# RainbowXXX/3DReconstruction

Hardware: AMD Instinct MI355X
Metric: BA LM-iters/sec + obs/sec, 1k cams/500k pts/5M obs; SIFT match pairs/sec (higher is better)
Workload: dtype f64; 1 GPU; C4 BA 1000 cams / 500000 pts / 5000000 obs, banded orbit visibility k=10, HuberLoss(4), gauge image 1, Ceres-default LM to termination per step; parallelism=landmark-sharded x1, all-reduce of the RCS, transport=none

## Files before the change

3dreconstruction_amd/_abi.py:

```python
import ctypes as C
import os

_HERE = os.path.dirname(os.path.abspath(__file__))
LIB_PATH = os.path.join(_HERE, "lib", "libsfmcore.so")

SFM_OK = 0
SFM_ERR_INVALID_ARG = -1
SFM_ERR_DEVICE = -2
SFM_ERR_NOT_FINITE = -3
SFM_ERR_UNSUPPORTED = -4
SFM_ERR_COMM = -5
SFM_ERR_OOM = -6
SFM_ERR_SOLVER = -7

SFM_TERM_CONVERGENCE = 0
SFM_TERM_NO_CONVERGENCE = 1
SFM_TERM_FAILURE = 2

SFM_CAM_PINHOLE = 0
SFM_CAM_SNAVELY = 1
SFM_CAM_RADIAL3 = 2

SFM_CTX_TUNE_HOST_MALLOC = 1
SFM_CTX_DIAG_NO_EXCHANGE = 2
SFM_CTX_DIAG_FAIL_SOLVE_WAIT = 4
SFM_CTX_TIME_KERNELS = 8
SFM_CTX_BA_DENSE_RCS = 1 << 4
SFM_CTX_BA_SEQ_BAND = 1 << 5
SFM_CTX_BA_TILE80 = 1 << 6
SFM_CTX_BA_SPLIT_REDUCE = 1 << 7
SFM_CTX_BA_SPLIT_BCR = 1 << 8
SFM_CTX_BA_NO_SPEC_GRAM = 1 << 10
SFM_CTX_DIAG_SPEC_ALWAYS = 1 << 11
SFM_CTX_BA_DENSE_CHAIN = 1 << 9


def SFM_CTX_BA_STEP_LANES(n):
    return {1: 1, 2: 2, 4: 3, 8: 4}[n] << 12


def SFM_CTX_BA_REDUCE_WAVES(n):
    return {1: 1, 2: 2, 4: 3}[n] << 15


SFM_RCS_BCR, SFM_RCS_DENSE, SFM_RCS_SEQ_BAND = 0, 1, 2

SFM_TRI_LINEAR, SFM_TRI_ROBUST = 0, 1
SFM_TRI_OK, SFM_TRI_SHORT, SFM_TRI_ANGLE, SFM_TRI_INFINITE = 0, 1, 2, 3

# ... 336 lines not shown
```

3dreconstruction_amd/csrc/ba_bcr.h:

```cpp
#pragma once
#include <hip/hip_runtime.h>

#include <vector>

#include "ba_kernels.h"

namespace sfm {

constexpr int kBcrM = 64;
constexpr int kBcrK = 10;

struct BcrArgs {
    int N = 0;
    int K = 0;
    int nrhs = 0;
    double *A = nullptr, *C = nullptr, *L = nullptr, *Wl = nullptr, *Wr = nullptr;
    double *R = nullptr, *Z = nullptr, *Y = nullptr, *part = nullptr, *fail = nullptr;
    unsigned* yflag = nullptr;
    unsigned long long* stamps = nullptr;
    bool split = false;
};

struct DenseArgs {
    int nt = 0;
    int64_t np = 0;
    double *A = nullptr, *X = nullptr, *b = nullptr, *y = nullptr, *x = nullptr, *fail = nullptr;
    unsigned* xflag = nullptr;
    unsigned* fflag = nullptr;
    unsigned long long* xg = nullptr;
    unsigned long long* stamps = nullptr;
    const int32_t* meta = nullptr;
    int nch = 0, ntask = 0;
    int64_t meta_words = 0;
    bool flow = false;
    bool chain = false;
};
size_t dense_flag_words(const DenseArgs& d);
void dense_setup(DenseArgs& d, const DevProblem& P);
std::vector<int32_t> dense_flow_plan(DenseArgs& d, const DevProblem& P, const std::vector<char>* exact = nullptr);
std::vector<char> dense_tile_pattern(const std::vector<ReduceTarget>& targets, int64_t nF, int nt);
size_t dense_doubles(const DenseArgs& d);
void dense_bind(DenseArgs& d, double* base);
void dense_solve(const DenseArgs& d, const DevProblem& P, double radius, hipStream_t s, unsigned epoch);

bool bcr_supported(const DevProblem& P);
void bcr_setup(BcrArgs& b, const DevProblem& P);
size_t bcr_doubles(const BcrArgs& b);
inline size_t bcr_y_granules(const BcrArgs& b) { return (size_t)b.N * 128; }
void bcr_bind(BcrArgs& b, double* base);
struct BcrCand {
    const double* extr;
    const double* intr;
    double* cand_extr;
    double* cand_intr;
    CamPre* cand_cp;
};
void bcr_solve(const BcrArgs& b, const DevProblem& P, double radius, hipStream_t s, unsigned epoch,
               const BcrCand& cand);

}
```

3dreconstruction_amd/csrc/ba_bcr.hip:

```cpp
#include <hip/hip_runtime.h>

#include <algorithm>
#include <cfloat>
#include <cmath>
#include <cstdlib>
#include <cstring>
#include <functional>
#include <type_traits>
#include <utility>

#include "ba_bcr.h"
#include "ba_cand.h"
#include "common.h"

#if defined(__HIP_DEVICE_COMPILE__) && !defined(__gfx950__)
#error "counter-form hand-offs (sc1 payloads + vmcnt drain + relaxed ticket) are written for gfx950 only"
#endif

namespace sfm {
namespace {

constexpr int M = kBcrM;
constexpr int LD = M + 1;
constexpr int NT = 256;
// ... 10 lines not shown

__device__ __forceinline__ int bcr_kM(const BcrArgs& b) { return b.K <= 9 ? 56 : b.K == 10 ? 60 : 64; }

__device__ __forceinline__ double clampd(double v, double lo, double hi) { return fmin(fmax(v, lo), hi); }

typedef __attribute__((address_space(1))) unsigned long long gu64;
typedef __attribute__((address_space(1))) unsigned gu32;
typedef __attribute__((address_space(1))) double gf64;
__device__ __forceinline__ void st_sc1(double* p, double v) {
    __hip_atomic_store((gf64*)p, v, __ATOMIC_RELAXED, __HIP_MEMORY_SCOPE_AGENT);
}
__device__ __forceinline__ double ld_sc1(const double* p) {
    return __hip_atomic_load((gf64*)p, __ATOMIC_RELAXED, __HIP_MEMORY_SCOPE_AGENT);
}

typedef double v4d __attribute__((ext_vector_type(4)));

__device__ __forceinline__ unsigned long long stamp() {
    unsigned long long t;
    asm volatile("s_memtime %0\n\ts_waitcnt lgkmcnt(0)" : "=s"(t)::"memory");
    return t;
}

__device__ __forceinline__ void wave_sync() {
    __builtin_amdgcn_fence(__ATOMIC_RELEASE, "wavefront");
    __builtin_amdgcn_wave_barrier();
    __builtin_amdgcn_fence(__ATOMIC_ACQUIRE, "wavefront");
}

__device__ __forceinline__ double rsqrt_nr(double d) {
    const double y = __builtin_amdgcn_rsq(d);
// ... 67 lines not shown
    __builtin_amdgcn_sched_barrier(0);
#pragma unroll
    for (int q = 0; q < 16; ++q)
        if (q < 14 || 4 * q < kM) acc = __builtin_amdgcn_mfma_f64_16x16x4f64(NEG ? -a[q] : a[q], b[q], acc, 0, 0, 0);
    return acc;
}
struct GTile {
    double v[16];
    __device__ __forceinline__ void fetch(const double* p, int ld) {
        const int lane = threadIdx.x & 63, i = lane & 15, kk = lane >> 4;
#pragma unroll
        for (int c = 0; c < 4; ++c)
#pragma unroll
            for (int j = 0; j < 4; ++j) v[4 * c + j] = p[(16 * c + 4 * j + kk) * ld + i];
    }
};
template <bool NEG, class PA>
__device__ __forceinline__ v4d mm_tr(v4d acc, PA A, int lda, int ar, const GTile& g, int kM) {
    const int lane = threadIdx.x & 63, i = lane & 15, kk = lane >> 4;
    double a[16];
#pragma unroll
    for (int q = 0; q < 16; ++q) a[q] = A[(4 * q + kk) * lda + ar + i];
    __builtin_amdgcn_sched_barrier(0);
#pragma unroll
    for (int q = 0; q < 16; ++q)
        if (q < 14 || 4 * q < kM)
            acc = __builtin_amdgcn_mfma_f64_16x16x4f64(NEG ? -a[q] : a[q], g.v[q], acc, 0, 0, 0);
    return acc;
}
template <bool NEG, class PB>
// ... 10 lines not shown
    return acc;
}
__device__ __forceinline__ lds_cd* L3(const double* p) { return (lds_cd*)p; }

__device__ __forceinline__ v4d tile_ld(const double* C, int ldc, int r0, int c0) {
    const int lane = threadIdx.x & 63, i = lane & 15, kk = lane >> 4;
    v4d v;
#pragma unroll
    for (int r = 0; r < 4; ++r) v[r] = C[(r0 + kk + 4 * r) * ldc + c0 + i];
    return v;
}
__device__ __forceinline__ void tile_st(double* C, int ldc, int r0, int c0, v4d v) {
    const int lane = threadIdx.x & 63, i = lane & 15, kk = lane >> 4;
#pragma unroll
    for (int r = 0; r < 4; ++r) C[(r0 + kk + 4 * r) * ldc + c0 + i] = v[r];
}
__device__ __forceinline__ v4d zero4() { return v4d{0.0, 0.0, 0.0, 0.0}; }

template <int NC, int R = M, int TH = NT>
__device__ __forceinline__ void load_tile(double* dst, int ld_dst, const double* __restrict__ src, int ld_src) {
    constexpr int n2 = R * NC / 2, per = (n2 + TH - 1) / TH;
    double2 v[per];
#pragma unroll
    for (int q = 0; q < per; ++q) {
        const int e = threadIdx.x + q * TH;
        if (e < n2) v[q] = *reinterpret_cast<const double2*>(src + (e / (NC / 2)) * ld_src + 2 * (e % (NC / 2)));
    }
#pragma unroll
    for (int q = 0; q < per; ++q) {
        const int e = threadIdx.x + q * TH;
// ... 1 lines not shown
            double* d = dst + (e / (NC / 2)) * ld_dst + 2 * (e % (NC / 2));
            d[0] = v[q].x;
            d[1] = v[q].y;
        }
    }
}
template <int NC, int R = M, int TH = NT>
struct TileFetch {
    static constexpr int n2 = R * NC / 2, per = (n2 + TH - 1) / TH;
    double2 v[per];
    __device__ __forceinline__ void fetch(const double* __restrict__ src, int ld_src) {
#pragma unroll
        for (int q = 0; q < per; ++q) {
            const int e = threadIdx.x + q * TH;
            if (e < n2) v[q] = *reinterpret_cast<const double2*>(src + (e / (NC / 2)) * ld_src + 2 * (e % (NC / 2)));
        }
    }
    __device__ __forceinline__ void put(double* dst, int ld_dst) const {
#pragma unroll
        for (int q = 0; q < per; ++q) {
            const int e = threadIdx.x + q * TH;
            if (e < n2) {
                double* d = dst + (e / (NC / 2)) * ld_dst + 2 * (e % (NC / 2));
                d[0] = v[q].x;
                d[1] = v[q].y;
            }
        }
    }
};
__device__ __forceinline__ void load_tiles2(double* d1, const double* __restrict__ s1, double* d2,
// ... 297 lines not shown
        const double lm = sqrt(clampd(cn, P.min_diag, P.max_diag) / radius);
        dmp = creal ? lm * lm : 0.0;
    }
    __device__ __forceinline__ double a(const DevProblem& P, int r, int c) const {
        const int ci = c0 + r / 6, rm = r % 6;
        const bool real = r < nreal && creal;
        const int d = ci >= cj ? ci - cj : cj - ci;
        const bool inband = real && d <= P.D;
        const int idx = ci >= cj ? ((ci * Dp + d) * 36 + rm * 6 + cm) : ((cj * Dp + d) * 36 + cm * 6 + rm);
        const double v = P.Sband[inband ? idx : 0];
        double x = inband ? v : 0.0;
        x = (real && r == c) ? x + dmp : x;
        return r >= nreal && r == c ? 1.0 : x;
    }
};
template <int TH>
__device__ __forceinline__ void pack_rows(const BcrArgs& b, const DevProblem& P, double radius, int I, int r0, int t) {
    double* A = b.A + (size_t)I * M * M + (size_t)r0 * M;
    double* R = b.R + (size_t)I * M * b.nrhs + (size_t)r0 * b.nrhs;
    static_assert(TH % M == 0, "a thread's column is fixed");
    constexpr int NA = 16 * M / TH;
    const BandCol col(b, P, radius, I, t % M);
    double va[NA];
#pragma unroll
    for (int q = 0; q < NA; ++q) {
        const int e = t + q * TH;
        va[q] = col.a(P, r0 + e / M, e % M);
    }
    static_assert(16 * 32 <= TH, "one R element per thread at most (nrhs <= 32)");
    const bool hasr = t < 16 * b.nrhs;
    const double vr = pack_r(b, P, I, r0 + t / b.nrhs, t % b.nrhs, hasr);
#pragma unroll
    for (int q = 0; q < NA; ++q) A[t + q * TH] = va[q];
    if (hasr) R[t] = vr;
}

__global__ void bcr_pack_kernel(BcrArgs b, DevProblem P, double radius) {
    const int I = blockIdx.x >> 4, rg = blockIdx.x & 15;
    double* A = b.A + (size_t)I * M * M;
    double* Cm = b.C + (size_t)I * M * M;
    double* R = b.R + (size_t)I * M * b.nrhs;
    {
        const int e = 4 * rg * M + threadIdx.x;
        const int r = e / M, c = e % M;
        A[e] = pack_a(b, P, radius, I, r, c);
        Cm[e] = pack_c(b, P, I, r, c);
    }
    for (int e = 4 * rg * b.nrhs + threadIdx.x; e < 4 * (rg + 1) * b.nrhs; e += NT)
        R[e] = pack_r(b, P, I, e / b.nrhs, e % b.nrhs);
// ... 37 lines not shown
    if (wv < 4) {
        v4d acc = tile_ld(Aj, M, 16 * w, 16 * v);
        if (hl) acc = mm_ll_rows<true, false, true>(acc, L3(Wa), LD, 16 * w, L3(Wa), LD, 16 * v, kM);
        if (hr) acc = mm_ll_rows<true, false, true>(acc, L3(Wb), LD, 16 * w, L3(Wb), LD, 16 * v, kM);
        tile_st(Aj, M, 16 * w, 16 * v, acc);
        return;
    }
    if (16 * v < b.nrhs) {
        double* Rj = b.R + (size_t)j * M * b.nrhs;
        v4d acc = tile_ld(Rj, b.nrhs, 16 * w, 16 * v);
        if (hl) acc = mm_ll_rows<true, false, true>(acc, L3(Wa), LD, 16 * w, L3(Za), ldr, 16 * v, kM);
        if (hr) acc = mm_ll_rows<true, false, true>(acc, L3(Wb), LD, 16 * w, L3(Zb), ldr, 16 * v, kM);
        tile_st(Rj, b.nrhs, 16 * w, 16 * v, acc);
    }
}

constexpr int NTL = 512, NWL = NTL / 64;

__device__ __forceinline__ void bcr_corner_body(const BcrArgs& b, const DevProblem& P, double radius, int I,
                                                bool z_fresh, bool part_done = false, unsigned tag = 0,
                                                const double* own = nullptr);
__device__ __forceinline__ void put_y(unsigned long long* g, int row, double v, unsigned epoch);
__device__ __forceinline__ void corner_put_lds(const DevProblem& P, const v4d& q00, double* dst) {
    constexpr int kQ = 17;
    const int lane = threadIdx.x & 63, i = lane & 15, kk = lane >> 4, na = P.iw * P.nintr;
#pragma unroll
    for (int r = 0; r < 4; ++r) {
        const int ga = kk + 4 * r, gc = i;
        if (ga >= 1 && ga <= na && gc <= na) dst[(ga - 1) * kQ + gc] = q00[r];
    }
// ... 5 lines not shown
    double* out = b.part + (size_t)I * 512;
    auto put = [&](const v4d& q, int r0, int c0) {
#pragma unroll
        for (int r = 0; r < 4; ++r) {
            const int ga = r0 + kk + 4 * r, gc = c0 + i;
            if (ga >= 1 && ga <= na && gc <= na) st_sc1(out + (ga - 1) * kQ + gc, q[r]);
        }
    };
    put(q00, 0, 0);
    if (ntc > 1) {
        put(q10, 16, 0);
        put(q11, 16, 16);
    }
}

template <bool TOP>
__global__ __launch_bounds__(NTL) void bcr_level_kernel(BcrArgs b, DevProblem P, double radius, int s, int n_odd,
                                                        unsigned epoch) {
    extern __shared__ __attribute__((aligned(16))) double sm[];
    int item, w;
    if constexpr (TOP) {
        if ((int)blockIdx.x >= 4) {
            bcr_corner_body(b, P, radius, (int)blockIdx.x - 3, false, false, epoch);
            return;
        }
        item = 0;
        w = blockIdx.x;
    } else {
        const int xcd = blockIdx.x & 7, q = blockIdx.x >> 3;
        item = xcd + 8 * (q >> 2);
        w = q & 3;
    }
    const int sp = s >> 1;
    if (!TOP && item >= n_odd) {
        const int j = 2 * s * (item - n_odd);
        if (sp > 0 && j < b.N) update_tile_rows<NTL>(b, sp, j, w, sm);
        return;
    }
    const int i = TOP ? 0 : s + 2 * s * item;
    if (i >= b.N) return;
    const int r = i + s, wave = threadIdx.x >> 6;
    const bool hr = !TOP && r < b.N, hz = 16 * w < b.nrhs;
    const int np3 = 6 * b.K - 48;
    const int kM = bcr_kM(b);
    constexpr int L16 = 17;
    double* A = sm;
    double* X = A + M * LD;
    double* Wa_l = X + M * LD;
    double* Wb_l = Wa_l + M * M;
    double* Cc = Wb_l + M * M;
    double* Cr = Cc + M * L16;
    double* Rc = Cr + 16 * LD;
    double* bad = Rc + M * L16;
    double* col = bad + 2;
    unsigned* pdone = reinterpret_cast<unsigned*>(col + 16);
    unsigned long long* st = (b.stamps && w == 0 && !TOP) ? b.stamps : nullptr;
    unsigned long long t0 = 0, t1 = 0;
    if (st) t0 = stamp();
    if (threadIdx.x == 0) bad[0] = 0.0;
    if (threadIdx.x < 4) pdone[threadIdx.x] = 0u;
    TileFetch<64, M, NTL> fa;
    TileFetch<16, M, NTL> frc;
    if (!TOP && sp == 0) {
        constexpr int QA = M * M / NTL, QC = M * 16 / NTL;
        double va[QA], vc[QC], vr[QC], vz[QC];
        const BandCol col(b, P, radius, i, threadIdx.x % M);
#pragma unroll
        for (int q = 0; q < QA; ++q) {
            const int e = threadIdx.x + q * NTL;
            va[q] = col.a(P, e / M, e % M);
        }
// ... 4 lines not shown
            vr[q] = pack_c(b, P, r, 16 * w + e / M, e % M, hr);
            vz[q] = pack_r(b, P, i, e / 16, 16 * w + e % 16, hz);
        }
#pragma unroll
        for (int q = 0; q < QA; ++q) {
            const int e = threadIdx.x + q * NTL;
            A[(e / M) * LD + e % M] = va[q];
        }
#pragma unroll
        for (int q = 0; q < QC; ++q) {
            const int e = threadIdx.x + q * NTL;
            Cc[(e / 16) * L16 + e % 16] = vc[q];
            Cr[(e / M) * LD + e % M] = vr[q];
            Rc[(e / 16) * L16 + e % 16] = vz[q];
        }
        pack_rows<NTL>(b, P, radius, i - 1, 16 * w, threadIdx.x);
        if (i + 1 == b.N - 1) pack_rows<NTL>(b, P, radius, i + 1, 16 * w, threadIdx.x);
    } else {
        TileFetch<64, M, NTL> fwa, fwb;
        const bool hwb = i + sp < b.N;
        if (!TOP) fwa.fetch(b.Wr + (size_t)(i - sp) * M * M, M);
        if (hwb) fwb.fetch(b.Wl + (size_t)(i + sp) * M * M, M);
        fa.fetch(b.A + (size_t)i * M * M, M);
        if (hz) frc.fetch(b.R + (size_t)i * M * b.nrhs + 16 * w, b.nrhs);
        if (!TOP) fwa.put(Wa_l, M);
        if (hwb) fwb.put(Wb_l, M);
        fa.put(A, LD);
        if (hz) frc.put(Rc, L16);
    }
    __syncthreads();
    if (st) {
        t1 = stamp();
        if (threadIdx.x == 0) atomicAdd(st + 5, t1 - t0);
    }
    {
    const bool upd = sp > 0;
    const int il = TOP ? i : i - sp, ir = i + sp;
    const bool hir = upd && ir < b.N;
    const double* Z1 = b.Z + (size_t)il * M * b.nrhs + 16 * w;
// ... 37 lines not shown
    auto bgR = [&](int v, const GTile& g1, const GTile& g2) {
        if (!hzu) return;
        v4d acc = tile_ld(Rc, L16, 16 * v, 0);
        if (!TOP) acc = mm_tr<true>(acc, L3(Wal), M, 16 * v, g1, kM);
        if (hir) acc = mm_tr<true>(acc, L3(Wbl), M, 16 * v, g2, kM);
        tile_st(Rc, L16, 16 * v, 0, acc);
    };
    auto bgC = [&](int v, const GTile& gl) {
        if (upd && !TOP) tile_st(Cc, L16, 16 * v, 0, mm_tr<true>(zero4(), L3(Wal), M, 16 * v, gl, kM));
    };
    auto bgCr = [&](int v, const GTile& gr) {
        if (hr && hir) tile_st(Cr, LD, 0, 16 * v, mm_rt<true>(zero4(), gr, L3(Wbl), M, 16 * v, kM));
    };
    auto fetch_z = [&](GTile& g1, GTile& g2) {
        if (!hzu) return;
        if (!TOP) g1.fetch(Z1, b.nrhs);
        if (hir) g2.fetch(Z2, b.nrhs);
    };
    auto fetch_wl = [&](GTile& g) {
        if (upd && !TOP) g.fetch(WL, M);
    };
    auto fetch_wr = [&](GTile& g) {
        if (hr && hir) g.fetch(WR, M);
    };
    auto pphase = [&](int k) {
        if (wave >= 3) return;
        if (wave >= 3 - k && k > w) return;
        if (wave < 3 - k) {
            const int ii = k + 1 + wave;
            tile_st(A, LD, 16 * ii, 16 * k,
                    tile_mm<false, true, false>(zero4(), L3(A), LD, 16 * ii, L3(X), LD, 16 * k, 16 * k, 16 * k + 16));
        } else {
            const int j = wave - (3 - k);
            tile_st(X, LD, 16 * k, 16 * j,
                    tile_mm<false, false, true>(zero4(), L3(X), LD, 16 * k, L3(X), LD, 16 * j, 16 * k, 16 * k + 16));
        }
    };
// ... 28 lines not shown
        } else if (hir) part = tile_mm<true, false, false>(part, L3(Wbl), M, 0, L3(Wbl), M, 0, 16 * v, 16 * v + 16);
        if (upd) tile_st(tile_at(1, kS0[wave][0], kS0[wave][1]), LD, 0, 0, part);
    }
    __syncthreads();
    double* const Wlg = b.Wl + (size_t)i * M * M;
    double* const Wrg = b.Wr + (size_t)i * M * M;
    double* const Zg = b.Z + (size_t)i * M * b.nrhs;
    auto fs_l = [&](double* B, int k) {
        v4d acc = tile_ld(B, L16, 16 * k, 0);
        acc = mm_ll<false, false, true>(acc, L3(A), LD, 16 * k, L3(B), L16, 0, 0, 16 * k);
        tile_st(B, L16, 16 * k, 0, acc);
    };
    auto gs_l = [&](double* B, int k, double* G, int ldg) {
        const v4d o = mm_ll<false, false, false>(zero4(), L3(X), LD, 16 * k, L3(B), L16, 0, 16 * k, 16 * k + 16);
        tile_st(B, L16, 16 * k, 0, o);
        tile_st(G, ldg, 16 * k, 16 * w, o);
        return o;
    };
    v4d qz = zero4();
    const bool q_here = TOP && w == 0 && gridDim.x > 4;
    auto fs_r = [&](int k) {
        v4d acc = tile_ld(Cr, LD, 0, 16 * k);
        acc = mm_ll<false, true, true>(acc, L3(Cr), LD, 0, L3(A), LD, 16 * k, 0, 16 * k);
        tile_st(Cr, LD, 0, 16 * k, acc);
    };
    auto gs_r = [&](int k) {
        const v4d o = tile_mm<false, true, false>(zero4(), L3(Cr), LD, 0, L3(X), LD, 16 * k, 16 * k, 16 * k + 16);
        tile_st(Cr, LD, 0, 16 * k, o);
        const int lane = threadIdx.x & 63, li = lane & 15, kk = lane >> 4;
#pragma unroll
        for (int q = 0; q < 4; ++q) Wrg[(16 * k + li) * M + 16 * w + kk + 4 * q] = o[q];
    };
    auto gs_k = [&](int k) {
        if (wave == 5) {
            if (!TOP) gs_l(Cc, k, Wlg, M);
        } else if (wave == 6 && hr) {
            gs_r(k);
        } else if (wave == 7 && hz) {
            const v4d o = gs_l(Rc, k, Zg, b.nrhs);
            if (q_here) {
#pragma unroll
                for (int r = 0; r < 4; ++r) qz = __builtin_amdgcn_mfma_f64_16x16x4f64(o[r], o[r], qz, 0, 0, 0);
            }
        }
    };
    auto fs_lk = [&](int k) {
// ... 126 lines not shown
    gs_k(3);
    if (q_here && wave == 7) corner_put_lds(P, qz, Cc);
    if (st && threadIdx.x == 0) {
        atomicAdd(st + 0, td);
        atomicAdd(st + 1, stamp() - tf0);
        atomicAdd(st + 7, tq);
        for (int q = 0; q < 8; ++q) atomicAdd(st + 8 + q, wmax[q]);
    }
    if (w == 3) {
        __syncthreads();
        store_x(NTL, threadIdx.x);
    }
    }
    if (threadIdx.x == 0 && bad[0] != 0.0) b.fail[0] = 1.0;
    if constexpr (TOP) {
        if (w == 0 && gridDim.x > 4) {
            __syncthreads();
            bcr_corner_body(b, P, radius, 0, true, true, epoch, Cc);
        }
        return;
    }
    if (st) {
        __syncthreads();
        if (threadIdx.x == 0) atomicAdd(st + 6, stamp() - t0);
    }
    if (st) {
        __syncthreads();
        if (threadIdx.x == 0) {
            atomicAdd(st + 2, t1 - t0);
            atomicAdd(st + 3, stamp() - t0);
            atomicAdd(st + 4, 1ull);
        }
    }
}

__device__ __forceinline__ void bcr_top_body(const BcrArgs& b, int sp, double* sm) {
    const int ldr = b.nrhs + 1, kM = bcr_kM(b);
    double* A = sm;
    double* X = A + M * LD;
    double* R = X + M * LD;
    double* T = R + M * ldr;
    double* Wb = T + M * ldr;
    double* Zb = Wb + M * LD;
    double* sc = Zb + M * ldr;
    double* bad = sc + 33;
    const int wave = threadIdx.x >> 6;
    const bool upd = sp > 0 && sp < b.N;
    if (threadIdx.x == 0) bad[0] = 0.0;
// ... 457 lines not shown
}

__global__ void bcr_verdict_kernel(BcrArgs b, DevProblem P) {
    P.scal[kScSolveFail] = solve_verdict(b.fail);
    reset_verdict(b);
}

}

bool bcr_supported(const DevProblem& P) { return P.D <= kBcrK && P.ncam > 0 && P.iw * P.nintr <= 16; }

void bcr_setup(BcrArgs& b, const DevProblem& P) {
    b.K = std::max(9, P.D);
    b.N = (P.ncam + b.K - 1) / b.K;
    b.nrhs = ((1 + P.iw * P.nintr) + 15) / 16 * 16;
}

size_t bcr_doubles(const BcrArgs& b) {
    const size_t mm = (size_t)b.N * M * M, mr = (size_t)b.N * M * b.nrhs;
    return 5 * mm + 3 * mr + 512 * ((size_t)b.N + 1) + 8 + ((size_t)b.N + 1) / 2 + 2;
}

void bcr_bind(BcrArgs& b, double* base) {
    const size_t mm = (size_t)b.N * M * M, mr = (size_t)b.N * M * b.nrhs;
    b.A = base; b.C = b.A + mm; b.L = b.C + mm; b.Wl = b.L + mm; b.Wr = b.Wl + mm;
    b.R = b.Wr + mm; b.Z = b.R + mr; b.Y = b.Z + mr;
    b.part = b.Y + mr; b.fail = b.part + 512 * ((size_t)b.N + 1);
    b.yflag = reinterpret_cast<unsigned*>(b.fail + 8);
}

void bcr_solve(const BcrArgs& b, const DevProblem& P, double radius, hipStream_t s, unsigned epoch,
               const BcrCand& cand) {
    if (b.N == 1) {
        hipLaunchKernelGGL(bcr_pack_kernel, dim3(16 * b.N), dim3(NT), 0, s, b, P, radius);
        SFM_HIP(hipGetLastError());
    }
    const size_t ldr = b.nrhs + 1;
    const size_t lds_odd = (2 * M * LD + 2 * M * M + 2 * M * 17 + 16 * LD + 20) * sizeof(double);
    const size_t lds_even = (2 * M * LD + 2 * M * ldr) * sizeof(double);
    const size_t lds_l = std::max(lds_odd, lds_even);
    const size_t lds_t = (3 * M * LD + 3 * M * ldr + 34) * sizeof(double);
    {
        const size_t cap = 160 * 1024;
        set_dyn_lds((const void*)bcr_level_kernel<false>, cap);
        set_dyn_lds((const void*)bcr_top_kernel, cap);
        set_dyn_lds((const void*)bcr_level_kernel<true>, lds_l);
    }
    int s_top = 1;
    for (int stride = 1; stride < b.N; stride *= 2) {
        const int n_odd = (b.N - stride + 2 * stride - 1) / (2 * stride);
        const int n_even = stride > 1 ? (b.N + 2 * stride - 1) / (2 * stride) : 0;
        hipLaunchKernelGGL(bcr_level_kernel<false>, dim3(32 * ((n_odd + n_even + 7) / 8)), dim3(NTL), lds_l, s, b, P,
                           radius, stride, n_odd, 0u);
        SFM_HIP(hipGetLastError());
        s_top = stride * 2;
    }
    const bool top_level = b.N >= 2 && b.nrhs == 16;
    if (top_level) {
        hipLaunchKernelGGL(bcr_level_kernel<true>, dim3(b.split ? 4 : 3 + b.N), dim3(NTL), lds_l, s, b, P, radius,
                           s_top, 1, epoch);
        SFM_HIP(hipGetLastError());
        if (b.split) {
            hipLaunchKernelGGL(bcr_corner_kernel, dim3(b.N), dim3(NT), 0, s, b, P, radius);
            SFM_HIP(hipGetLastError());
        }
    } else if (!b.split) {
        set_dyn_lds((const void*)bcr_top_corner_kernel, 156 * 1024);
        hipLaunchKernelGGL(bcr_top_corner_kernel, dim3(b.N), dim3(NTL), lds_t, s, b, P, radius, s_top / 2);
        SFM_HIP(hipGetLastError());
    } else {
        hipLaunchKernelGGL(bcr_top_kernel, dim3(1), dim3(NTL), lds_t, s, b, s_top / 2);
        SFM_HIP(hipGetLastError());
        hipLaunchKernelGGL(bcr_corner_kernel, dim3(b.N), dim3(NT), 0, s, b, P, radius);
// ... 1105 lines not shown
```

3dreconstruction_amd/csrc/ba_solver.cpp:

```cpp
#include <hip/hip_runtime.h>

#include <algorithm>
#include <atomic>
#include <cfloat>
#include <chrono>
#include <cmath>
#include <cstdlib>
#include <cstdio>
#include <cstring>
#include <limits>
#include <memory>
#include <vector>
#include <unordered_map>
#include <thread>
#include <mutex>

#include "ba_bcr.h"
#include "ba_kernels.h"
#include "ba_order.h"
#include "ba_plan.h"
#include "ba_wash.h"
#include "common.h"
#include "../include/sfm/pool.hpp"

// ... 377 lines not shown
            pl->dense.stamps = pl->bcr_stamps.p;
        }
    }
    if (pl->use_bcr) {
        BcrArgs tmp;
        bcr_setup(tmp, P);
        P.n_fblk = tmp.N + 1;
    } else {
        P.n_fblk = ba_cand_blocks(P);
    }
    pl->part_f.alloc(3 * (size_t)P.n_fblk);
    P.part_f = pl->part_f.p;
    if (pl->use_bcr) {
        bcr_setup(pl->bcr, P);
        pl->bcr.split = (ctx->flags & SFM_CTX_BA_SPLIT_BCR) != 0;
        pl->bcr_buf.alloc(bcr_doubles(pl->bcr));
        bcr_bind(pl->bcr, pl->bcr_buf.p);
        SFM_HIP(hipMemsetAsync(pl->bcr.fail, 0, 8 * sizeof(double) + sizeof(unsigned) * (size_t)pl->bcr.N, s));
        SFM_HIP(hipMemsetAsync(pl->bcr.Y, 0, sizeof(double) * bcr_y_granules(pl->bcr), s));
        SFM_HIP(hipMemsetAsync(pl->bcr.part + (size_t)pl->bcr.N * 512, 0, 512 * sizeof(double), s));
        if (std::getenv("SFM_BCR_STAMPS")) {
            pl->bcr_stamps.alloc(16);
            pl->bcr_stamps.zero(s);
            pl->bcr.stamps = pl->bcr_stamps.p;
        }
    }
    if (std::getenv("SFM_SCHUR_STAMPS")) pl->stamps.alloc(6 * std::max<size_t>(h.chunks.size(), 1));
}

bool create_plan(sfm_ba_plan* pl, const sfm_ba_problem& prob, const double* extr, const double* intr,
                 const double* X, sfm_ba_plan* seed = nullptr, const GrowPrev* prev = nullptr) {
    PhaseTimer tm("create_plan");
    if (!plan_host(pl, prob, seed, prev, tm)) return false;
// ... 696 lines not shown
```

include/sfmcore.h:

```cpp
#ifndef SFMCORE_H
#define SFMCORE_H

#include <stdint.h>

#ifdef __cplusplus
extern "C" {
#endif
#pragma GCC visibility push(default)

#define SFM_OK                 0
#define SFM_ERR_INVALID_ARG   -1
#define SFM_ERR_DEVICE        -2
#define SFM_ERR_NOT_FINITE    -3
#define SFM_ERR_UNSUPPORTED   -4
#define SFM_ERR_COMM          -5
#define SFM_ERR_OOM           -6
#define SFM_ERR_SOLVER        -7

const char* sfm_version(void);
const char* sfm_last_error(void);

typedef struct sfm_ctx sfm_ctx;

typedef int32_t (*sfm_allreduce_fn)(void* user, double* buf, int64_t n, int32_t op);
// ... 10 lines not shown

#define SFM_CTX_TUNE_HOST_MALLOC 1
#define SFM_CTX_DIAG_NO_EXCHANGE 2
#define SFM_CTX_DIAG_FAIL_SOLVE_WAIT 4
#define SFM_CTX_TIME_KERNELS 8
#define SFM_CTX_DIAG_SPEC_ALWAYS (1 << 11)
#define SFM_CTX_BA_DENSE_RCS      (1 << 4)
#define SFM_CTX_BA_SEQ_BAND       (1 << 5)
#define SFM_CTX_BA_TILE80         (1 << 6)
#define SFM_CTX_BA_SPLIT_REDUCE   (1 << 7)
#define SFM_CTX_BA_SPLIT_BCR      (1 << 8)
#define SFM_CTX_BA_DENSE_CHAIN    (1 << 9)
#define SFM_CTX_BA_NO_SPEC_GRAM   (1 << 10)
#define SFM_CTX_BA_STEP_LANES(n)  (((n) == 8 ? 4 : (n) == 4 ? 3 : (n) == 2 ? 2 : (n) == 1 ? 1 : 7) << 12)
#define SFM_CTX_BA_REDUCE_WAVES(n) (((n) == 4 ? 3 : (n) == 2 ? 2 : (n) == 1 ? 1 : 7) << 15)

int sfm_comm_unique_id(uint8_t* out128);
int sfm_ctx_create(const sfm_ctx_opts* opts, sfm_ctx** out);
int sfm_ctx_destroy(sfm_ctx* ctx);
int sfm_ctx_synchronize(sfm_ctx* ctx);

typedef struct sfm_ba_problem {
    int32_t n_img;
    int32_t n_intr;
    int64_t n_pt;
    int64_t n_obs;
    const int64_t* pt_offsets;
    const int32_t* obs_img;
    const double*  obs_uv;
    const int32_t* img_intr;
// ... 374 lines not shown
```

Before: 1151 LM-iters/s.

## Fuse BCR level launches into one dataflow kernel with per-tile flag hand-offs

Replaces the per-level sequence of block-cyclic-reduction kernel launches (plus the top/corner launch) with a single persistent kernel. Blocks of each level spin on per-row tags written with agent-scope relaxed stores, and producers drain vmcnt before publishing. This removes the launch gaps and full-grid serialization between levels so later levels can start as soon as their inputs are ready. The risks are spin-wait deadlock if blocks are not co-resident in order, extra sc1 load/store traffic that bypasses caching, and a fallback flag to restore the old path.

```diff
diff --git a/3dreconstruction_amd/_abi.py b/3dreconstruction_amd/_abi.py
--- a/3dreconstruction_amd/_abi.py
+++ b/3dreconstruction_amd/_abi.py
@@ -33,6 +33,7 @@
 SFM_CTX_BA_NO_SPEC_GRAM = 1 << 10
 SFM_CTX_DIAG_SPEC_ALWAYS = 1 << 11
 SFM_CTX_BA_DENSE_CHAIN = 1 << 9
+SFM_CTX_BA_BCR_LEVEL_LAUNCHES = 1 << 18
 
 
 def SFM_CTX_BA_STEP_LANES(n):
diff --git a/3dreconstruction_amd/csrc/ba_bcr.h b/3dreconstruction_amd/csrc/ba_bcr.h
--- a/3dreconstruction_amd/csrc/ba_bcr.h
+++ b/3dreconstruction_amd/csrc/ba_bcr.h
@@ -9,6 +9,7 @@
 
 constexpr int kBcrM = 64;
 constexpr int kBcrK = 10;
+constexpr int kBcrFlowLevels = 8;
 
 struct BcrArgs {
     int N = 0;
@@ -19,6 +20,10 @@
     unsigned* yflag = nullptr;
     unsigned long long* stamps = nullptr;
     bool split = false;
+    unsigned* ftag = nullptr;
+    int fl_nlev = 0;
+    int fl_base[kBcrFlowLevels + 3] = {};
+    bool level_launches = false;
 };
 
 struct DenseArgs {
@@ -47,6 +52,9 @@
 void bcr_setup(BcrArgs& b, const DevProblem& P);
 size_t bcr_doubles(const BcrArgs& b);
 inline size_t bcr_y_granules(const BcrArgs& b) { return (size_t)b.N * 128; }
+inline size_t bcr_flag_doubles(const BcrArgs& b) {
+    return (8 + ((size_t)b.N + 1) / 2 + 2 + 4 * (size_t)b.N + 1) & ~(size_t)1;
+}
 void bcr_bind(BcrArgs& b, double* base);
 struct BcrCand {
     const double* extr;
diff --git a/3dreconstruction_amd/csrc/ba_bcr.hip b/3dreconstruction_amd/csrc/ba_bcr.hip
--- a/3dreconstruction_amd/csrc/ba_bcr.hip
+++ b/3dreconstruction_amd/csrc/ba_bcr.hip
@@ -48,7 +48,44 @@
     return __hip_atomic_load((gf64*)p, __ATOMIC_RELAXED, __HIP_MEMORY_SCOPE_AGENT);
 }
 
+typedef unsigned v4u __attribute__((ext_vector_type(4)));
+__device__ __forceinline__ __amdgpu_buffer_rsrc_t sc1_rsrc(const double* base, int bytes) {
+    return __builtin_amdgcn_make_buffer_rsrc(const_cast<double*>(base), 0, bytes, 0x00027000);
+}
+__device__ __forceinline__ double2 ld2_sc1(__amdgpu_buffer_rsrc_t rsrc, int off) {
+    return __builtin_bit_cast(double2, __builtin_amdgcn_raw_buffer_load_b128(rsrc, off, 0, 16));
+}
+
 typedef double v4d __attribute__((ext_vector_type(4)));
+
+__device__ __forceinline__ unsigned flow_tag(unsigned epoch, int lv) { return (epoch << 4) | (unsigned)lv; }
+__device__ __forceinline__ unsigned* flow_tag_o(const BcrArgs& b, int i) { return b.ftag + 4 * (size_t)i; }
+__device__ __forceinline__ unsigned* flow_tag_e(const BcrArgs& b, int j) { return b.ftag + 4 * (size_t)(b.N + j); }
+__device__ __forceinline__ void flow_wait(const BcrArgs& b, const unsigned* g0, int n0, const unsigned* g1,
+                                          const unsigned* g2, unsigned want) {
+    const int lane = threadIdx.x & 63, g = lane >> 2, q = lane & 3;
+    const unsigned* p = nullptr;
+    if (g == 0 && g0 && q < n0) p = g0 + q;
+    if (g == 1 && g1) p = g1 + q;
+    if (g == 2 && g2) p = g2 + q;
+    for (unsigned spins = 0;; ++spins) {
+        bool ok = true;
+        if (p) ok = __hip_atomic_load((gu32*)p, __ATOMIC_RELAXED, __HIP_MEMORY_SCOPE_AGENT) == want;
+        if (__all(ok)) break;
+        __builtin_amdgcn_s_sleep(1);
+        if (spins > (1u << 22)) {
+            if (lane == 0) st_sc1(b.fail + 1, 1.0);
+            break;
+        }
+    }
+}
+__device__ __forceinline__ void flow_drain() {
+    asm volatile("s_waitcnt vmcnt(0)" ::: "memory");
+    __syncthreads();
+}
+__device__ __forceinline__ void flow_put(unsigned* p, unsigned tag) {
+    __hip_atomic_store((gu32*)p, tag, __ATOMIC_RELAXED, __HIP_MEMORY_SCOPE_AGENT);
+}
 
 __device__ __forceinline__ unsigned long long stamp() {
     unsigned long long t;
@@ -146,6 +183,13 @@
 #pragma unroll
             for (int j = 0; j < 4; ++j) v[4 * c + j] = p[(16 * c + 4 * j + kk) * ld + i];
     }
+    __device__ __forceinline__ void fetch_sc1(const double* p, int ld) {
+        const int lane = threadIdx.x & 63, i = lane & 15, kk = lane >> 4;
+#pragma unroll
+        for (int c = 0; c < 4; ++c)
+#pragma unroll
+            for (int j = 0; j < 4; ++j) v[4 * c + j] = ld_sc1(p + (16 * c + 4 * j + kk) * ld + i);
+    }
 };
 template <bool NEG, class PA>
 __device__ __forceinline__ v4d mm_tr(v4d acc, PA A, int lda, int ar, const GTile& g, int kM) {
@@ -186,6 +230,18 @@
     const int lane = threadIdx.x & 63, i = lane & 15, kk = lane >> 4;
 #pragma unroll
     for (int r = 0; r < 4; ++r) C[(r0 + kk + 4 * r) * ldc + c0 + i] = v[r];
+}
+__device__ __forceinline__ v4d tile_ld_sc1(const double* C, int ldc, int r0, int c0) {
+    const int lane = threadIdx.x & 63, i = lane & 15, kk = lane >> 4;
+    v4d v;
+#pragma unroll
+    for (int r = 0; r < 4; ++r) v[r] = ld_sc1(C + (r0 + kk + 4 * r) * ldc + c0 + i);
+    return v;
+}
+__device__ __forceinline__ void tile_st_sc1(double* C, int ldc, int r0, int c0, v4d v) {
+    const int lane = threadIdx.x & 63, i = lane & 15, kk = lane >> 4;
+#pragma unroll
+    for (int r = 0; r < 4; ++r) st_sc1(C + (r0 + kk + 4 * r) * ldc + c0 + i, v[r]);
 }
 __device__ __forceinline__ v4d zero4() { return v4d{0.0, 0.0, 0.0, 0.0}; }
 
@@ -217,6 +273,14 @@
         for (int q = 0; q < per; ++q) {
             const int e = threadIdx.x + q * TH;
             if (e < n2) v[q] = *reinterpret_cast<const double2*>(src + (e / (NC / 2)) * ld_src + 2 * (e % (NC / 2)));
+        }
+    }
+    __device__ __forceinline__ void fetch_sc1(const double* src, int ld_src) {
+        const __amdgpu_buffer_rsrc_t rs = sc1_rsrc(src, ((R - 1) * ld_src + NC) * (int)sizeof(double));
+#pragma unroll
+        for (int q = 0; q < per; ++q) {
+            const int e = threadIdx.x + q * TH;
+            if (e < n2) v[q] = ld2_sc1(rs, ((e / (NC / 2)) * ld_src + 2 * (e % (NC / 2))) * (int)sizeof(double));
         }
     }
     __device__ __forceinline__ void put(double* dst, int ld_dst) const {
@@ -544,7 +608,7 @@
         return r >= nreal && r == c ? 1.0 : x;
     }
 };
-template <int TH>
+template <int TH, bool FLOW = false>
 __device__ __forceinline__ void pack_rows(const BcrArgs& b, const DevProblem& P, double radius, int I, int r0, int t) {
     double* A = b.A + (size_t)I * M * M + (size_t)r0 * M;
     double* R = b.R + (size_t)I * M * b.nrhs + (size_t)r0 * b.nrhs;
@@ -561,8 +625,14 @@
     const bool hasr = t < 16 * b.nrhs;
     const double vr = pack_r(b, P, I, r0 + t / b.nrhs, t % b.nrhs, hasr);
 #pragma unroll
-    for (int q = 0; q < NA; ++q) A[t + q * TH] = va[q];
-    if (hasr) R[t] = vr;
+    for (int q = 0; q < NA; ++q) {
+        if constexpr (FLOW) st_sc1(A + t + q * TH, va[q]);
+        else A[t + q * TH] = va[q];
+    }
+    if (hasr) {
+        if constexpr (FLOW) st_sc1(R + t, vr);
+        else R[t] = vr;
+    }
 }
 
 __global__ void bcr_pack_kernel(BcrArgs b, DevProblem P, double radius) {
@@ -630,6 +700,60 @@
         tile_st(Rj, b.nrhs, 16 * w, 16 * v, acc);
     }
 }
+template <int TH>
+__device__ void update_tile_rows_flow(const BcrArgs& b, int s, int j, int w, double* sm, unsigned epoch, int lv) {
+    const int kM = bcr_kM(b);
+    constexpr int ldr = 17;
+    double* Wa = sm;
+    double* Wb = Wa + M * LD;
+    double* Za = Wb + M * LD;
+    double* Zb = Za + M * ldr;
+    const int il = j - s, ir = j + s, wv = threadIdx.x >> 6, v = wv & 3;
+    const bool hl = il >= 0, hr = ir < b.N;
+    const unsigned want = flow_tag(epoch, lv - 1);
+    double* Aj = b.A + (size_t)j * M * M;
+    double* Rj = b.R + (size_t)j * M * 16;
+    if (wv == 0) flow_wait(b, flow_tag_e(b, j) + w, 1, nullptr, nullptr, want);
+    __syncthreads();
+    v4d acc = zero4();
+    if (wv < 4) acc = tile_ld_sc1(Aj, M, 16 * w, 16 * v);
+    else if (v == 0) acc = tile_ld_sc1(Rj, 16, 16 * w, 0);
+    if (wv == 0)
+        flow_wait(b, nullptr, 0, hl ? flow_tag_o(b, il) : nullptr, hr ? flow_tag_o(b, ir) : nullptr, want);
+    __syncthreads();
+    {
+        TileFetch<64, M, TH> fwa, fwb;
+        TileFetch<16, M, TH> fza, fzb;
+        if (hl) {
+            fwa.fetch_sc1(b.Wr + (size_t)il * M * M, M);
+            fza.fetch_sc1(b.Z + (size_t)il * M * 16, 16);
+        }
+        if (hr) {
+            fwb.fetch_sc1(b.Wl + (size_t)ir * M * M, M);
+            fzb.fetch_sc1(b.Z + (size_t)ir * M * 16, 16);
+        }
+        if (hl) {
+            fwa.put(Wa, LD);
+            fza.put(Za, ldr);
+        }
+        if (hr) {
+            fwb.put(Wb, LD);
+            fzb.put(Zb, ldr);
+        }
+    }
+    __syncthreads();
+    if (wv < 4) {
+        if (hl) acc = mm_ll_rows<true, false, true>(acc, L3(Wa), LD, 16 * w, L3(Wa), LD, 16 * v, kM);
+        if (hr) acc = mm_ll_rows<true, false, true>(acc, L3(Wb), LD, 16 * w, L3(Wb), LD, 16 * v, kM);
+        tile_st_sc1(Aj, M, 16 * w, 16 * v, acc);
+    } else if (v == 0) {
+        if (hl) acc = mm_ll_rows<true, false, true>(acc, L3(Wa), LD, 16 * w, L3(Za), ldr, 0, kM);
+        if (hr) acc = mm_ll_rows<true, false, true>(acc, L3(Wb), LD, 16 * w, L3(Zb), ldr, 0, kM);
+        tile_st_sc1(Rj, 16, 16 * w, 0, acc);
+    }
+    flow_drain();
+    if (threadIdx.x == 0) flow_put(flow_tag_e(b, j) + w, flow_tag(epoch, lv));
+}
 
 constexpr int NTL = 512, NWL = NTL / 64;
 
@@ -665,27 +789,16 @@
     }
 }
 
-template <bool TOP>
-__global__ __launch_bounds__(NTL) void bcr_level_kernel(BcrArgs b, DevProblem P, double radius, int s, int n_odd,
-                                                        unsigned epoch) {
-    extern __shared__ __attribute__((aligned(16))) double sm[];
-    int item, w;
-    if constexpr (TOP) {
-        if ((int)blockIdx.x >= 4) {
-            bcr_corner_body(b, P, radius, (int)blockIdx.x - 3, false, false, epoch);
-            return;
-        }
-        item = 0;
-        w = blockIdx.x;
-    } else {
-        const int xcd = blockIdx.x & 7, q = blockIdx.x >> 3;
-        item = xcd + 8 * (q >> 2);
-        w = q & 3;
-    }
+template <bool TOP, bool FLOW>
+__device__ __forceinline__ void bcr_level_body(const BcrArgs& b, const DevProblem& P, double radius, int s, int n_odd,
+                                               unsigned epoch, int item, int w, bool fused, int lv, double* sm) {
     const int sp = s >> 1;
     if (!TOP && item >= n_odd) {
         const int j = 2 * s * (item - n_odd);
-        if (sp > 0 && j < b.N) update_tile_rows<NTL>(b, sp, j, w, sm);
+        if (sp > 0 && j < b.N) {
+            if constexpr (FLOW) update_tile_rows_flow<NTL>(b, sp, j, w, sm, epoch, lv);
+            else update_tile_rows<NTL>(b, sp, j, w, sm);
+        }
         return;
     }
     const int i = TOP ? 0 : s + 2 * s * item;
@@ -705,7 +818,7 @@
     double* bad = Rc + M * L16;
     double* col = bad + 2;
     unsigned* pdone = reinterpret_cast<unsigned*>(col + 16);
-    unsigned long long* st = (b.stamps && w == 0 && !TOP) ? b.stamps : nullptr;
+    unsigned long long* st = (!FLOW && b.stamps && w == 0 && !TOP) ? b.stamps : nullptr;
     unsigned long long t0 = 0, t1 = 0;
     if (st) t0 = stamp();
     if (threadIdx.x == 0) bad[0] = 0.0;
@@ -740,15 +853,29 @@
             Cr[(e / M) * LD + e % M] = vr[q];
             Rc[(e / 16) * L16 + e % 16] = vz[q];
         }
-        pack_rows<NTL>(b, P, radius, i - 1, 16 * w, threadIdx.x);
-        if (i + 1 == b.N - 1) pack_rows<NTL>(b, P, radius, i + 1, 16 * w, threadIdx.x);
+        pack_rows<NTL, FLOW>(b, P, radius, i - 1, 16 * w, threadIdx.x);
+        if (i + 1 == b.N - 1) pack_rows<NTL, FLOW>(b, P, radius, i + 1, 16 * w, threadIdx.x);
     } else {
         TileFetch<64, M, NTL> fwa, fwb;
         const bool hwb = i + sp < b.N;
-        if (!TOP) fwa.fetch(b.Wr + (size_t)(i - sp) * M * M, M);
-        if (hwb) fwb.fetch(b.Wl + (size_t)(i + sp) * M * M, M);
-        fa.fetch(b.A + (size_t)i * M * M, M);
-        if (hz) frc.fetch(b.R + (size_t)i * M * b.nrhs + 16 * w, b.nrhs);
+        if constexpr (FLOW) {
+            const unsigned want = flow_tag(epoch, lv - 1);
+            if (wave == 0) flow_wait(b, flow_tag_e(b, i), 4, nullptr, nullptr, want);
+            __syncthreads();
+            fa.fetch_sc1(b.A + (size_t)i * M * M, M);
+            if (hz) frc.fetch_sc1(b.R + (size_t)i * M * b.nrhs + 16 * w, b.nrhs);
+            if (wave == 0)
+                flow_wait(b, nullptr, 0, TOP ? nullptr : flow_tag_o(b, i - sp), hwb ? flow_tag_o(b, i + sp) : nullptr,
+                          want);
+            __syncthreads();
+            if (!TOP) fwa.fetch_sc1(b.Wr + (size_t)(i - sp) * M * M, M);
+            if (hwb) fwb.fetch_sc1(b.Wl + (size_t)(i + sp) * M * M, M);
+        } else {
+            if (!TOP) fwa.fetch(b.Wr + (size_t)(i - sp) * M * M, M);
+            if (hwb) fwb.fetch(b.Wl + (size_t)(i + sp) * M * M, M);
+            fa.fetch(b.A + (size_t)i * M * M, M);
+            if (hz) frc.fetch(b.R + (size_t)i * M * b.nrhs + 16 * w, b.nrhs);
+        }
         if (!TOP) fwa.put(Wa_l, M);
         if (hwb) fwb.put(Wb_l, M);
         fa.put(A, LD);
@@ -816,13 +943,26 @@
     };
     auto fetch_z = [&](GTile& g1, GTile& g2) {
         if (!hzu) return;
+        if constexpr (FLOW) {
+            if (!TOP) g1.fetch_sc1(Z1, b.nrhs);
+            if (hir) g2.fetch_sc1(Z2, b.nrhs);
+            return;
+        }
         if (!TOP) g1.fetch(Z1, b.nrhs);
         if (hir) g2.fetch(Z2, b.nrhs);
     };
     auto fetch_wl = [&](GTile& g) {
+        if constexpr (FLOW) {
+            if (upd && !TOP) g.fetch_sc1(WL, M);
+            return;
+        }
         if (upd && !TOP) g.fetch(WL, M);
     };
     auto fetch_wr = [&](GTile& g) {
+        if constexpr (FLOW) {
+            if (hr && hir) g.fetch_sc1(WR, M);
+            return;
+        }
         if (hr && hir) g.fetch(WR, M);
     };
     auto pphase = [&](int k) {
@@ -881,11 +1021,12 @@
     auto gs_l = [&](double* B, int k, double* G, int ldg) {
         const v4d o = mm_ll<false, false, false>(zero4(), L3(X), LD, 16 * k, L3(B), L16, 0, 16 * k, 16 * k + 16);
         tile_st(B, L16, 16 * k, 0, o);
-        tile_st(G, ldg, 16 * k, 16 * w, o);
+        if constexpr (FLOW && !TOP) tile_st_sc1(G, ldg, 16 * k, 16 * w, o);
+        else tile_st(G, ldg, 16 * k, 16 * w, o);
         return o;
     };
     v4d qz = zero4();
-    const bool q_here = TOP && w == 0 && gridDim.x > 4;
+    const bool q_here = TOP && w == 0 && fused;
     auto fs_r = [&](int k) {
         v4d acc = tile_ld(Cr, LD, 0, 16 * k);
         acc = mm_ll<false, true, true>(acc, L3(Cr), LD, 0, L3(A), LD, 16 * k, 0, 16 * k);
@@ -896,7 +1037,10 @@
         tile_st(Cr, LD, 0, 16 * k, o);
         const int lane = threadIdx.x & 63, li = lane & 15, kk = lane >> 4;
 #pragma unroll
-        for (int q = 0; q < 4; ++q) Wrg[(16 * k + li) * M + 16 * w + kk + 4 * q] = o[q];
+        for (int q = 0; q < 4; ++q) {
+            if constexpr (FLOW) st_sc1(Wrg + (16 * k + li) * M + 16 * w + kk + 4 * q, o[q]);
+            else Wrg[(16 * k + li) * M + 16 * w + kk + 4 * q] = o[q];
+        }
     };
     auto gs_k = [&](int k) {
         if (wave == 5) {
@@ -1053,9 +1197,21 @@
     }
     if (threadIdx.x == 0 && bad[0] != 0.0) b.fail[0] = 1.0;
     if constexpr (TOP) {
-        if (w == 0 && gridDim.x > 4) {
+        if (w == 0 && fused) {
             __syncthreads();
             bcr_corner_body(b, P, radius, 0, true, true, epoch, Cc);
+        }
+        return;
+    }
+    if constexpr (FLOW) {
+        flow_drain();
+        if (threadIdx.x == 0) {
+            const unsigned tag = flow_tag(epoch, lv);
+            flow_put(flow_tag_o(b, i) + w, tag);
+            if (sp == 0) {
+                flow_put(flow_tag_e(b, i - 1) + w, tag);
+                if (i + 1 == b.N - 1) flow_put(flow_tag_e(b, i + 1) + w, tag);
+            }
         }
         return;
     }
@@ -1071,6 +1227,49 @@
             atomicAdd(st + 4, 1ull);
         }
     }
+}
+
+template <bool TOP>
+__global__ __launch_bounds__(NTL) void bcr_level_kernel(BcrArgs b, DevProblem P, double radius, int s, int n_odd,
+                                                        unsigned epoch) {
+    extern __shared__ __attribute__((aligned(16))) double sm[];
+    int item, w;
+    if constexpr (TOP) {
+        if ((int)blockIdx.x >= 4) {
+            bcr_corner_body(b, P, radius, (int)blockIdx.x - 3, false, false, epoch);
+            return;
+        }
+        item = 0;
+        w = blockIdx.x;
+    } else {
+        const int xcd = blockIdx.x & 7, q = blockIdx.x >> 3;
+        item = xcd + 8 * (q >> 2);
+        w = q & 3;
+    }
+    bcr_level_body<TOP, false>(b, P, radius, s, n_odd, epoch, item, w, gridDim.x > 4, 0, sm);
+}
+
+__global__ __launch_bounds__(NTL) void bcr_flow_kernel(BcrArgs b, DevProblem P, double radius, unsigned epoch) {
+    extern __shared__ __attribute__((aligned(16))) double sm[];
+    const int g = blockIdx.x, nlev = b.fl_nlev;
+    if (g >= b.fl_base[nlev + 1]) {
+        bcr_level_body<true, true>(b, P, radius, 1 << nlev, 1, epoch, 0, g - b.fl_base[nlev + 1], true, nlev + 1, sm);
+        return;
+    }
+    if (g >= b.fl_base[nlev]) {
+        const int I = g - b.fl_base[nlev] + 1;
+        if (threadIdx.x < 64)
+            flow_wait(b, flow_tag_o(b, I), 1, nullptr, nullptr, flow_tag(epoch, __builtin_ctz((unsigned)I) + 1));
+        __syncthreads();
+        bcr_corner_body(b, P, radius, I, true, false, epoch);
+        return;
+    }
+    int l = 0;
+    while (g >= b.fl_base[l + 1]) ++l;
+    const int x = g - b.fl_base[l], xcd = x & 7, q = x >> 3;
+    const int s = 1 << l;
+    bcr_level_body<false, true>(b, P, radius, s, (b.N + s - 1) >> (l + 1), epoch, xcd + 8 * (q >> 2), q & 3, false,
+                                l + 1, sm);
 }
 
 __device__ __forceinline__ void bcr_top_body(const BcrArgs& b, int sp, double* sm) {
@@ -1558,11 +1757,27 @@
     b.K = std::max(9, P.D);
     b.N = (P.ncam + b.K - 1) / b.K;
     b.nrhs = ((1 + P.iw * P.nintr) + 15) / 16 * 16;
+    b.fl_nlev = 0;
+    int nlev = 0;
+    for (int stride = 1; stride < b.N; stride *= 2) ++nlev;
+    if (b.N >= 2 && b.nrhs == 16 && nlev <= kBcrFlowLevels) {
+        int base = 0, l = 0;
+        for (int stride = 1; stride < b.N; stride *= 2, ++l) {
+            const int n_odd = (b.N - stride + 2 * stride - 1) / (2 * stride);
+            const int n_even = stride > 1 ? (b.N + 2 * stride - 1) / (2 * stride) : 0;
+            b.fl_base[l] = base;
+            base += 32 * ((n_odd + n_even + 7) / 8);
+        }
+        b.fl_base[nlev] = base;
+        b.fl_base[nlev + 1] = base + b.N - 1;
+        b.fl_base[nlev + 2] = base + b.N - 1 + 4;
+        b.fl_nlev = nlev;
+    }
 }
 
 size_t bcr_doubles(const BcrArgs& b) {
     const size_t mm = (size_t)b.N * M * M, mr = (size_t)b.N * M * b.nrhs;
-    return 5 * mm + 3 * mr + 512 * ((size_t)b.N + 1) + 8 + ((size_t)b.N + 1) / 2 + 2;
+    return 5 * mm + 3 * mr + 512 * ((size_t)b.N + 1) + bcr_flag_doubles(b);
 }
 
 void bcr_bind(BcrArgs& b, double* base) {
@@ -1571,6 +1786,7 @@
     b.R = b.Wr + mm; b.Z = b.R + mr; b.Y = b.Z + mr;
     b.part = b.Y + mr; b.fail = b.part + 512 * ((size_t)b.N + 1);
     b.yflag = reinterpret_cast<unsigned*>(b.fail + 8);
+    b.ftag = reinterpret_cast<unsigned*>(b.fail + 8 + ((size_t)b.N + 1) / 2 + 2);
 }
 
 void bcr_solve(const BcrArgs& b, const DevProblem& P, double radius, hipStream_t s, unsigned epoch,
@@ -1590,8 +1806,16 @@
         set_dyn_lds((const void*)bcr_top_kernel, cap);
         set_dyn_lds((const void*)bcr_level_kernel<true>, lds_l);
     }
+    const bool top_level = b.N >= 2 && b.nrhs == 16;
+    const bool flow = top_level && b.fl_nlev > 0 && !b.split && !b.level_launches && !b.stamps;
     int s_top = 1;
-    for (int stride = 1; stride < b.N; stride *= 2) {
+    if (flow) {
+        set_dyn_lds((const void*)bcr_flow_kernel, lds_l);
+        hipLaunchKernelGGL(bcr_flow_kernel, dim3(b.fl_base[b.fl_nlev + 2]), dim3(NTL), lds_l, s, b, P, radius, epoch);
+        SFM_HIP(hipGetLastError());
+        s_top = 1 << b.fl_nlev;
+    }
+    for (int stride = 1; stride < b.N && !flow; stride *= 2) {
         const int n_odd = (b.N - stride + 2 * stride - 1) / (2 * stride);
         const int n_even = stride > 1 ? (b.N + 2 * stride - 1) / (2 * stride) : 0;
         hipLaunchKernelGGL(bcr_level_kernel<false>, dim3(32 * ((n_odd + n_even + 7) / 8)), dim3(NTL), lds_l, s, b, P,
@@ -1599,8 +1823,8 @@
         SFM_HIP(hipGetLastError());
         s_top = stride * 2;
     }
-    const bool top_level = b.N >= 2 && b.nrhs == 16;
-    if (top_level) {
+    if (flow) {
+    } else if (top_level) {
         hipLaunchKernelGGL(bcr_level_kernel<true>, dim3(b.split ? 4 : 3 + b.N), dim3(NTL), lds_l, s, b, P, radius,
                            s_top, 1, epoch);
         SFM_HIP(hipGetLastError());
diff --git a/3dreconstruction_amd/csrc/ba_solver.cpp b/3dreconstruction_amd/csrc/ba_solver.cpp
--- a/3dreconstruction_amd/csrc/ba_solver.cpp
+++ b/3dreconstruction_amd/csrc/ba_solver.cpp
@@ -415,9 +415,10 @@
     if (pl->use_bcr) {
         bcr_setup(pl->bcr, P);
         pl->bcr.split = (ctx->flags & SFM_CTX_BA_SPLIT_BCR) != 0;
+        pl->bcr.level_launches = (ctx->flags & SFM_CTX_BA_BCR_LEVEL_LAUNCHES) != 0;
         pl->bcr_buf.alloc(bcr_doubles(pl->bcr));
         bcr_bind(pl->bcr, pl->bcr_buf.p);
-        SFM_HIP(hipMemsetAsync(pl->bcr.fail, 0, 8 * sizeof(double) + sizeof(unsigned) * (size_t)pl->bcr.N, s));
+        SFM_HIP(hipMemsetAsync(pl->bcr.fail, 0, sizeof(double) * bcr_flag_doubles(pl->bcr), s));
         SFM_HIP(hipMemsetAsync(pl->bcr.Y, 0, sizeof(double) * bcr_y_granules(pl->bcr), s));
         SFM_HIP(hipMemsetAsync(pl->bcr.part + (size_t)pl->bcr.N * 512, 0, 512 * sizeof(double), s));
         if (std::getenv("SFM_BCR_STAMPS")) {
diff --git a/include/sfmcore.h b/include/sfmcore.h
--- a/include/sfmcore.h
+++ b/include/sfmcore.h
@@ -48,6 +48,7 @@
 #define SFM_CTX_BA_NO_SPEC_GRAM   (1 << 10)
 #define SFM_CTX_BA_STEP_LANES(n)  (((n) == 8 ? 4 : (n) == 4 ? 3 : (n) == 2 ? 2 : (n) == 1 ? 1 : 7) << 12)
 #define SFM_CTX_BA_REDUCE_WAVES(n) (((n) == 4 ? 3 : (n) == 2 ? 2 : (n) == 1 ? 1 : 7) << 15)
+#define SFM_CTX_BA_BCR_LEVEL_LAUNCHES (1 << 18)
 
 int sfm_comm_unique_id(uint8_t* out128);
 int sfm_ctx_create(const sfm_ctx_opts* opts, sfm_ctx** out);
```

Result: no change. 1156 LM-iters/s, median of 6 (+0.4%).
